# PrimeIntellect-ai/prime

Measured on AMD Instinct MI355X. Metric: tokens_per_sec, higher is better.
Workload: dtype bf16; 1 GPU; model=intellect_10b, global_batch=8, seq_len=2048, parallelism=diloco1_h100_int8ring

## Files before the change

### prime_amd/ops/csrc/attention.hip

```cpp
#include "common.h"
#include <stdlib.h>
#include <type_traits>

typedef __attribute__((ext_vector_type(8))) short short8;
typedef __attribute__((ext_vector_type(4))) float f32x4;
typedef __attribute__((address_space(3))) char lds_char;
typedef __attribute__((address_space(3))) void lds_void;
typedef __attribute__((address_space(1))) const void g_void;

__device__ __forceinline__ short8 ld8(const bf16* p) {
  return *reinterpret_cast<const short8*>(p);
}

__device__ __forceinline__ f32x4 mfma16(short8 a, short8 b, f32x4 c) {
  return __builtin_amdgcn_mfma_f32_16x16x32_bf16(a, b, c, 0, 0, 0);
}

__device__ __forceinline__ float grp16_max(float x) {
#pragma unroll
  for (int off = 1; off < 16; off <<= 1) x = fmaxf(x, __shfl_xor(x, off, 64));
  return x;
}
__device__ __forceinline__ float grp16_sum(float x) {
#pragma unroll
  for (int off = 1; off < 16; off <<= 1) x += __shfl_xor(x, off, 64);
  return x;
}

#define NEG_INF (-1e30f)


template <int ROWS, int COLS, int NT = 256>
__device__ __forceinline__ void stage_tile(const bf16* __restrict__ gbase,
                                           int64_t row_stride, bf16* lds_tile,
                                           int tid) {
  constexpr int UNITS = ROWS * COLS / 8;
  constexpr int UPR = COLS / 8;
  static_assert(UNITS % NT == 0, "tile not divisible by block lanes");
#pragma unroll
  for (int i = 0; i < UNITS / NT; ++i) {
    const int u = i * NT + tid;
    const int row = u / UPR;
    const int colb = ((u % UPR) * 16) ^ ((row & 7) << 4);
    const bf16* src = gbase + (int64_t)row * row_stride + colb / 2;
    const int wid = tid >> 6;
    lds_void* dst = (lds_void*)((lds_char*)lds_tile + i * (NT * 16) + wid * 1024);
    __builtin_amdgcn_global_load_lds((g_void*)src, dst, 16, 0, 0);
  }
}

template <int COLS>
__device__ __forceinline__ short8 ld8_swz(const bf16* lds_tile, int row,
                                          int colb) {
  return *reinterpret_cast<const short8*>(
      reinterpret_cast<const char*>(lds_tile) + row * (COLS * 2) +
      (colb ^ ((row & 7) << 4)));
}

template <int COLS>
__device__ __forceinline__ void st16_swz(bf16* lds_tile, int row, int col,
                                         bf16 v) {
  *reinterpret_cast<bf16*>(reinterpret_cast<char*>(lds_tile) + row * (COLS * 2) +
                           ((col * 2) ^ ((row & 7) << 4))) = v;
}

__device__ __forceinline__ void wave_lds_fence() {
  asm volatile("s_waitcnt lgkmcnt(0)" ::: "memory");
  __builtin_amdgcn_sched_barrier(0);
}

__device__ __forceinline__ int doc_clamp(int v, int hi) {
  return v < 0 ? 0 : (v > hi ? hi : v);
}

template <int D, int NW, bool DOC = false>
__global__ __launch_bounds__(512) void flash_fwd_kernel(
    const bf16* __restrict__ Q, const bf16* __restrict__ K,
    const bf16* __restrict__ Vt, bf16* __restrict__ O, float* __restrict__ lse,
    int B, int H, int Hkv, int S, float scale, int causal,
    int64_t sqb, int64_t sqs, int64_t sqh,
    int64_t skb, int64_t sks, int64_t skh,
    const int* __restrict__ doc) {
  constexpr int DS = D / 32;
  constexpr int DT = D / 16;
  constexpr int QT = NW * 16;
  const int n_qt = S / QT;
  const int bh = blockIdx.x / n_qt;
  const int qt = n_qt - 1 - (blockIdx.x - bh * n_qt);
  const int b = bh / H, h = bh - b * H;
  const int hkv = h / (H / Hkv);
  const int wid = threadIdx.x >> 6;
  const int lane = threadIdx.x & 63;
  const int lg = lane >> 4, li = lane & 15;
  const int q0 = qt * QT + wid * 16;

  const bf16* Qb = Q + b * sqb + h * sqh;
  const bf16* Kb = K + b * skb + hkv * skh;
  const bf16* Vtb = Vt + ((int64_t)(b * Hkv + hkv) * D) * S;

  __shared__ bf16 k_lds[64 * D];
  __shared__ bf16 vt_lds[D * 64];
  __shared__ bf16 p_lds_all[NW][16 * 64];
  bf16* p_lds = p_lds_all[wid];

  short8 qf[DS];
#pragma unroll
  for (int ds = 0; ds < DS; ++ds)
    qf[ds] = ld8(Qb + (int64_t)(q0 + li) * sqs + ds * 32 + lg * 8);

  float m[4], l[4];
  f32x4 o_acc[DT];
#pragma unroll
  for (int r = 0; r < 4; ++r) { m[r] = NEG_INF; l[r] = 0.f; }
#pragma unroll
  for (int dt = 0; dt < DT; ++dt) o_acc[dt] = f32x4{0.f, 0.f, 0.f, 0.f};

  const int kv_end = causal ? (qt * QT + QT) : S;
  int kv_begin = 0, my_kv_begin = 0, row_ds[4];
  if (DOC) {
    const int* doc_b = doc + (int64_t)b * S;
    kv_begin = doc_clamp(doc_b[qt * QT], qt * QT) & ~63;
    my_kv_begin = doc_clamp(doc_b[q0], q0) & ~63;
#pragma unroll
    for (int r = 0; r < 4; ++r) row_ds[r] = doc_b[q0 + lg * 4 + r];
  }
  for (int kv = kv_begin; kv < kv_end; kv += 64) {
    __syncthreads();
    stage_tile<64, D, NW * 64>(Kb + (int64_t)kv * sks, sks, k_lds, threadIdx.x);
    stage_tile<D, 64, NW * 64>(Vtb + kv, S, vt_lds, threadIdx.x);
    __syncthreads();
    if (DOC && kv < my_kv_begin) continue;

    f32x4 s[4];
#pragma unroll
    for (int sub = 0; sub < 4; ++sub) {
      f32x4 acc{0.f, 0.f, 0.f, 0.f};
#pragma unroll
      for (int ds = 0; ds < DS; ++ds)
        acc = mfma16(qf[ds], ld8_swz<D>(k_lds, sub * 16 + li, ds * 64 + lg * 16), acc);
      s[sub] = acc;
    }
    float alpha[4];
#pragma unroll
    for (int r = 0; r < 4; ++r) {
      const int qg = q0 + lg * 4 + r;
      float tmax = NEG_INF;
#pragma unroll
      for (int sub = 0; sub < 4; ++sub) {
        float v = s[sub][r] * scale;
        if (causal && (kv + sub * 16 + li) > qg) v = NEG_INF;
        if (DOC && (kv + sub * 16 + li) < row_ds[r]) v = NEG_INF;
        s[sub][r] = v;
        tmax = fmaxf(tmax, v);
      }
      tmax = grp16_max(tmax);
      const float mnew = fmaxf(m[r], tmax);
      alpha[r] = (mnew == m[r]) ? 1.f : __expf(m[r] - mnew);
      float psum = 0.f;
#pragma unroll
      for (int sub = 0; sub < 4; ++sub) {
        const float p = (DOC && s[sub][r] <= NEG_INF)
                            ? 0.f : __expf(s[sub][r] - mnew);
        s[sub][r] = p;
        psum += p;
      }
      l[r] = l[r] * alpha[r] + grp16_sum(psum);
      m[r] = mnew;
    }
    float amin = 1.f;
#pragma unroll
    for (int r = 0; r < 4; ++r) amin = fminf(amin, alpha[r]);
    if (__ballot(amin < 1.f)) {
#pragma unroll
      for (int dt = 0; dt < DT; ++dt)
#pragma unroll
        for (int r = 0; r < 4; ++r) o_acc[dt][r] *= alpha[r];
    }
#pragma unroll
    for (int sub = 0; sub < 4; ++sub)
#pragma unroll
      for (int r = 0; r < 4; ++r)
        st16_swz<64>(p_lds, lg * 4 + r, sub * 16 + li, f2bf(s[sub][r]));
    wave_lds_fence();
#pragma unroll
    for (int dt = 0; dt < DT; ++dt)
#pragma unroll
      for (int ks = 0; ks < 2; ++ks)
        o_acc[dt] = mfma16(ld8_swz<64>(p_lds, li, ks * 64 + lg * 16),
                           ld8_swz<64>(vt_lds, dt * 16 + li, ks * 64 + lg * 16),
                           o_acc[dt]);
  }
#pragma unroll
  for (int r = 0; r < 4; ++r) {
    const float inv = (l[r] > 0.f) ? 1.f / l[r] : 0.f;
    const int qg = q0 + lg * 4 + r;
    bf16* orow = O + (((int64_t)(b * S + qg)) * H + h) * D;
#pragma unroll
    for (int dt = 0; dt < DT; ++dt)
      orow[dt * 16 + li] = f2bf(o_acc[dt][r] * inv);
    if (li == 0)
      lse[((int64_t)(b * S + qg)) * H + h] = m[r] + __logf(fmaxf(l[r], 1e-30f));
  }
}


typedef __attribute__((ext_vector_type(16))) float f32x16;

__device__ __forceinline__ f32x16 mfma32(short8 a, short8 b, f32x16 c) {
  return __builtin_amdgcn_mfma_f32_32x32x16_bf16(a, b, c, 0, 0, 0);
}

__device__ __forceinline__ unsigned cvt_pk_bf16(float lo_, float hi_) {
  unsigned r;
  asm("v_cvt_pk_bf16_f32 %0, %1, %2" : "=v"(r) : "v"(lo_), "v"(hi_));
  return r;
}

__device__ __forceinline__ void permlane32_swap(unsigned& a, unsigned& b) {
  asm volatile("v_permlane32_swap_b32 %0, %1" : "+v"(a), "+v"(b));
}

template <int D, bool DOC = false>
__global__ __launch_bounds__(512, 2) void flash_fwd_v5_kernel(
    const bf16* __restrict__ Q, const bf16* __restrict__ K,
    const bf16* __restrict__ Vt, bf16* __restrict__ O, float* __restrict__ lse,
    int B, int H, int Hkv, int S, float scale, int causal,
    int64_t sqb, int64_t sqs, int64_t sqh,
    int64_t skb, int64_t sks, int64_t skh,
    const int* __restrict__ doc) {
  constexpr int DSL = D / 16;
  constexpr int DT32 = D / 32;
  const int n_qt = S / 256;
  const int nwg = gridDim.x;
  int vb = blockIdx.x;
  if ((nwg & 7) == 0) vb = (blockIdx.x & 7) * (nwg >> 3) + (blockIdx.x >> 3);
  const int bh = vb / n_qt;
  const int qt = n_qt - 1 - (vb - bh * n_qt);
  const int b = bh / H, h = bh - b * H;
  const int hkv = h / (H / Hkv);
  const int wid = threadIdx.x >> 6;
  const int lane = threadIdx.x & 63;
  const int lo = lane & 31, hi = lane >> 5;
  const int q0w = qt * 256 + wid * 32;

  const bf16* Qb = Q + b * sqb + h * sqh;
  const bf16* Kb = K + b * skb + hkv * skh;
  const bf16* Vtb = Vt + ((int64_t)(b * Hkv + hkv) * D) * S;

  __shared__ bf16 k_lds[2][64 * D];
  __shared__ bf16 vt_lds[2][D * 64];
  __shared__ float bcast_all[8][32];
  float* bcast = bcast_all[wid];

  short8 qf[DSL];
#pragma unroll
  for (int ds = 0; ds < DSL; ++ds) {
    const bf16* src = Qb + (int64_t)(q0w + lo) * sqs + ds * 16 + hi * 8;
    short8 raw = ld8(src);
    short8 sc;
#pragma unroll
    for (int j = 0; j < 8; ++j) {
      bf16 v = reinterpret_cast<const bf16*>(&raw)[j];
      reinterpret_cast<bf16*>(&sc)[j] = f2bf(bf2f(v) * scale);
    }
    qf[ds] = sc;
  }

  float m_run = NEG_INF, l_run = 0.f;
  f32x16 o_acc[DT32];
#pragma unroll
  for (int dt = 0; dt < DT32; ++dt)
#pragma unroll
    for (int r = 0; r < 16; ++r) o_acc[dt][r] = 0.f;

  const int kv_end = causal ? (qt * 256 + 256) : S;
  const int my_kv_end = causal ? (q0w + 32) : S;
  int kv_begin = 0, my_kv_begin = 0, my_ds = 0, my_ds_last = 0;
  if (DOC) {
    const int* doc_b = doc + (int64_t)b * S;
    kv_begin = doc_clamp(doc_b[qt * 256], qt * 256) & ~63;
    my_kv_begin = doc_clamp(doc_b[q0w], q0w) & ~63;
    my_ds = doc_b[q0w + lo];
    my_ds_last = doc_b[q0w + 31];
  }
  stage_tile<64, D, 512>(Kb + (int64_t)kv_begin * sks, sks, k_lds[0], threadIdx.x);
  stage_tile<D, 64, 512>(Vtb + kv_begin, S, vt_lds[0], threadIdx.x);
  int idx = 0;
  for (int kv = kv_begin, kt = 0; kv < kv_end; kv += 64, ++kt) {
    idx = kt % 2;
    __syncthreads();
    if (kv + 64 < kv_end) {
      stage_tile<64, D, 512>(Kb + (int64_t)(kv + 64) * sks, sks,
                             k_lds[(kt + 1) % 2], threadIdx.x);
      stage_tile<D, 64, 512>(Vtb + kv + 64, S, vt_lds[(kt + 1) % 2],
                             threadIdx.x);
    }
    if (kv >= my_kv_end) continue;
    if (DOC && kv < my_kv_begin) continue;

    f32x16 st[2];
#pragma unroll
    for (int t = 0; t < 2; ++t) {
#pragma unroll
      for (int r = 0; r < 16; ++r) st[t][r] = 0.f;
#pragma unroll
      for (int ds = 0; ds < DSL; ++ds) {
        const short8 kf = ld8_swz<D>(k_lds[idx], t * 32 + lo, ds * 32 + hi * 16);
        st[t] = mfma32(kf, qf[ds], st[t]);
      }
    }
    float tmax = NEG_INF;
    if (DOC && kv < my_ds_last) {
#pragma unroll
      for (int t = 0; t < 2; ++t)
#pragma unroll
        for (int r = 0; r < 16; ++r) {
          const int kg = kv + t * 32 + (r & 3) + 8 * (r >> 2) + 4 * hi;
          if (kg < my_ds) st[t][r] = NEG_INF;
        }
    }
#pragma unroll
    for (int t = 0; t < 2; ++t)
#pragma unroll
      for (int r = 0; r < 16; ++r) {
        const int kg = kv + t * 32 + (r & 3) + 8 * (r >> 2) + 4 * hi;
        if (causal && kg > q0w + lo) st[t][r] = NEG_INF;
        tmax = fmaxf(tmax, st[t][r]);
      }
    tmax = fmaxf(tmax, __shfl_xor(tmax, 32, 64));
    const float thr = 8.f;
    float alpha = 1.f;
    if (__ballot(tmax > m_run + thr)) {
      const float mnew = fmaxf(m_run, tmax);
      alpha = __expf(m_run - mnew);
      m_run = mnew;
      if (hi == 0) bcast[lo] = alpha;
      wave_lds_fence();
#pragma unroll
      for (int dt = 0; dt < DT32; ++dt)
#pragma unroll
        for (int r = 0; r < 16; ++r)
          o_acc[dt][r] *= bcast[(r & 3) + 8 * (r >> 2) + 4 * hi];
    }
    float psum = 0.f;
#pragma unroll
    for (int t = 0; t < 2; ++t)
#pragma unroll
      for (int r = 0; r < 16; ++r) {
        const float pv = (st[t][r] <= NEG_INF) ? 0.f : __expf(st[t][r] - m_run);
        st[t][r] = pv;
        psum += pv;
      }
    psum += __shfl_xor(psum, 32, 64);
    l_run = l_run * alpha + psum;

    short8 pa[2 * 2];
#pragma unroll
    for (int t = 0; t < 2; ++t) {
#pragma unroll
      for (int kst = 0; kst < 2; ++kst) {
        const int g0 = 4 * (2 * kst), g1 = 4 * (2 * kst + 1);
        unsigned x0 = cvt_pk_bf16(st[t][g0 + 0], st[t][g0 + 1]);
        unsigned x1 = cvt_pk_bf16(st[t][g0 + 2], st[t][g0 + 3]);
        unsigned y0 = cvt_pk_bf16(st[t][g1 + 0], st[t][g1 + 1]);
        unsigned y1 = cvt_pk_bf16(st[t][g1 + 2], st[t][g1 + 3]);
        permlane32_swap(x0, y0);
        permlane32_swap(x1, y1);
        short8 frag;
        reinterpret_cast<unsigned*>(&frag)[0] = x0;
        reinterpret_cast<unsigned*>(&frag)[1] = x1;
        reinterpret_cast<unsigned*>(&frag)[2] = y0;
        reinterpret_cast<unsigned*>(&frag)[3] = y1;
        pa[t * 2 + kst] = frag;
      }
    }
#pragma unroll
    for (int dt = 0; dt < DT32; ++dt)
#pragma unroll
      for (int ks = 0; ks < 4; ++ks)
        o_acc[dt] = mfma32(pa[ks],
                           ld8_swz<64>(vt_lds[idx], dt * 32 + lo, ks * 32 + hi * 16),
                           o_acc[dt]);
  }
  if (hi == 0) bcast[lo] = (l_run > 0.f) ? 1.f / l_run : 0.f;
  wave_lds_fence();
#pragma unroll
  for (int r = 0; r < 16; ++r) {
    const int qr = (r & 3) + 8 * (r >> 2) + 4 * hi;
    const float inv = bcast[qr];
    bf16* orow = O + (((int64_t)(b * S + q0w + qr)) * H + h) * D;
#pragma unroll
    for (int dt = 0; dt < DT32; ++dt)
      orow[dt * 32 + lo] = f2bf(o_acc[dt][r] * inv);
  }
  if (hi == 0)
    lse[((int64_t)(b * S + q0w + lo)) * H + h] = m_run + __logf(fmaxf(l_run, 1e-30f));
}

__global__ void attn_delta_kernel(const bf16* __restrict__ dO,
                                  const bf16* __restrict__ O,
                                  float* __restrict__ delta, int64_t rows,
                                  int D, const float* __restrict__ lse,
                                  float* __restrict__ rowc_t, int S, int H) {
  const int64_t row0 = (int64_t)blockIdx.x * (blockDim.x >> 6) + (threadIdx.x >> 6);
  const int lane = threadIdx.x & 63;
  for (int64_t r = row0; r < rows; r += (int64_t)gridDim.x * (blockDim.x >> 6)) {
    float acc = 0.f;
    for (int i = lane * 2; i < D; i += 128) {
      acc += bf2f(dO[r * D + i]) * bf2f(O[r * D + i]);
      acc += bf2f(dO[r * D + i + 1]) * bf2f(O[r * D + i + 1]);
    }
    acc = wave_reduce_sum(acc);
    if (lane == 0) {
      delta[r] = acc;
      if (rowc_t) {
        const int64_t bs = r / H;
        const int h = (int)(r - bs * H);
        const int64_t bb = bs / S;
        const int s = (int)(bs - bb * S);
        const int64_t t = (bb * H + h) * S + s;
        rowc_t[t] = lse[r];
        rowc_t[rows + t] = acc;
      }
    }
  }
}

template <int D>
__global__ __launch_bounds__(256) void attn_delta_dot_kernel(
    const bf16* __restrict__ dO, const bf16* __restrict__ O,
    const float* __restrict__ lse, float* __restrict__ delta,
    float* __restrict__ rowc_t, bf16* __restrict__ dOt, int S, int H,
    int64_t rows) {
  constexpr int LPR = D / 8;
  constexpr int RPP = 256 / LPR;
  constexpr int NP = 64 / RPP;
  constexpr int TPD = D + 8;
  __shared__ __attribute__((aligned(16))) bf16 tile[64][TPD];
  __shared__ float sdelta[64];
  int idx = blockIdx.x;
  const int h = idx % H; idx /= H;
  const int n_st = S / 64;
  const int st = idx % n_st;
  const int b = idx / n_st;
  const int t = threadIdx.x;
  const int m = t % LPR, rr = t / LPR;
  const int64_t tok0 = (int64_t)b * S + st * 64;
  const int64_t tcol = ((int64_t)b * H + h) * S + st * 64;

  short8 vdo[NP], vo[NP];
#pragma unroll
  for (int p = 0; p < NP; ++p) {
    const int64_t off = ((tok0 + p * RPP + rr) * H + h) * D + m * 8;
    vdo[p] = *reinterpret_cast<const short8*>(dO + off);
    vo[p] = *reinterpret_cast<const short8*>(O + off);
  }
  float lv = 0.f;
  if (t >= 64 && t < 128) lv = lse[(tok0 + (t - 64)) * H + h];

#pragma unroll
  for (int p = 0; p < NP; ++p) {
    const int row = p * RPP + rr;
    *reinterpret_cast<short8*>(&tile[row][m * 8]) = vdo[p];
    const bf16* a = reinterpret_cast<const bf16*>(&vdo[p]);
    const bf16* c = reinterpret_cast<const bf16*>(&vo[p]);
    float q[4];
#pragma unroll
    for (int i = 0; i < 4; ++i) {
      float acc = 0.f;
      acc += bf2f(a[2 * i]) * bf2f(c[2 * i]);
      acc += bf2f(a[2 * i + 1]) * bf2f(c[2 * i + 1]);
      q[i] = acc;
    }
#pragma unroll
    for (int i = 0; i < 4; ++i) {
      if (D == 64) q[i] = q[i] + 0.f;
      else q[i] += __shfl_down(q[i], 8, 64);
    }
#pragma unroll
    for (int off = 4; off > 0; off >>= 1)
#pragma unroll
      for (int i = 0; i < 4; ++i) q[i] += __shfl_down(q[i], off, 64);
    if (m == 0) sdelta[row] = (q[0] + q[2]) + (q[1] + q[3]);
  }
  __syncthreads();
  if (t < 64) {
    const float d = sdelta[t];
    delta[(tok0 + t) * H + h] = d;
    rowc_t[rows + tcol + t] = d;
  } else if (t < 128) {
    rowc_t[tcol + (t - 64)] = lv;
  }
  bf16* dbase = dOt + ((int64_t)b * H + h) * D * S + st * 64;
#pragma unroll
  for (int i = 0; i < D / 32; ++i) {
    const int u = i * 256 + t;
    const int d = u >> 3, s8 = (u & 7) * 8;
    short8 v;
#pragma unroll
    for (int j = 0; j < 8; ++j)
      reinterpret_cast<short*>(&v)[j] =
          reinterpret_cast<const short*>(&tile[s8 + j][d])[0];
    *reinterpret_cast<short8*>(dbase + (int64_t)d * S + s8) = v;
  }
}

template <int D, bool DOC = false>
__global__ __launch_bounds__(512, 2) void flash_bwd_dq_v5_kernel(
    const bf16* __restrict__ Q, const bf16* __restrict__ K,
    const bf16* __restrict__ V, const bf16* __restrict__ Kt,
    const bf16* __restrict__ dO, const float* __restrict__ lse,
    const float* __restrict__ delta, bf16* __restrict__ dQ, int B, int H,
    int Hkv, int S, float scale, int causal,
    int64_t sqb, int64_t sqs, int64_t sqh,
    int64_t skb, int64_t sks, int64_t skh,
    int64_t svb, int64_t svs, int64_t svh,
    const int* __restrict__ doc) {
  constexpr int DSL = D / 16;
  constexpr int DT32 = D / 32;
  const int n_qt = S / 256;
  const int nwg = gridDim.x;
  int vb = blockIdx.x;
  if ((nwg & 7) == 0) vb = (blockIdx.x & 7) * (nwg >> 3) + (blockIdx.x >> 3);
  const int bh = vb / n_qt;
  const int qt = n_qt - 1 - (vb - bh * n_qt);
  const int b = bh / H, h = bh - b * H;
  const int hkv = h / (H / Hkv);
  const int wid = threadIdx.x >> 6;
  const int lane = threadIdx.x & 63;
  const int lo = lane & 31, hi = lane >> 5;
  const int q0w = qt * 256 + wid * 32;

  const bf16* Qb = Q + b * sqb + h * sqh;
  const bf16* Kb = K + b * skb + hkv * skh;
  const bf16* Vb = V + b * svb + hkv * svh;
  const bf16* Ktb = Kt + ((int64_t)(b * Hkv + hkv) * D) * S;
  const bf16* dOb = dO + ((int64_t)b * S * H + h) * D;
  const float* lse_b = lse + (int64_t)b * S * H + h;
  const float* dl_b = delta + (int64_t)b * S * H + h;

  __shared__ bf16 k_lds[2][64 * D];
  __shared__ bf16 v_lds[2][64 * D];
  __shared__ bf16 kt_lds[2][D * 64];

  short8 qf[DSL], dof[DSL];
#pragma unroll
  for (int ds = 0; ds < DSL; ++ds) {
    const bf16* src = Qb + (int64_t)(q0w + lo) * sqs + ds * 16 + hi * 8;
    short8 raw = ld8(src);
    short8 sc;
#pragma unroll
    for (int j = 0; j < 8; ++j) {
      bf16 v = reinterpret_cast<const bf16*>(&raw)[j];
      reinterpret_cast<bf16*>(&sc)[j] = f2bf(bf2f(v) * scale);
    }
    qf[ds] = sc;
    dof[ds] = ld8(dOb + (int64_t)(q0w + lo) * H * D + ds * 16 + hi * 8);
  }
  const float lse_q = lse_b[(int64_t)(q0w + lo) * H];
  const float dl_q = dl_b[(int64_t)(q0w + lo) * H];

  f32x16 dq_acc[DT32];
#pragma unroll
  for (int dt = 0; dt < DT32; ++dt)
#pragma unroll
    for (int r = 0; r < 16; ++r) dq_acc[dt][r] = 0.f;

  const int kv_end = causal ? (qt * 256 + 256) : S;
  const int my_kv_end = causal ? (q0w + 32) : S;
  int kv_begin = 0, my_kv_begin = 0, my_ds = 0;
  if (DOC) {
    const int* doc_b = doc + (int64_t)b * S;
    kv_begin = doc_clamp(doc_b[qt * 256], qt * 256) & ~63;
    my_kv_begin = doc_clamp(doc_b[q0w], q0w) & ~63;
    my_ds = doc_b[q0w + lo];
  }
  stage_tile<64, D, 512>(Kb + (int64_t)kv_begin * sks, sks, k_lds[0], threadIdx.x);
  stage_tile<64, D, 512>(Vb + (int64_t)kv_begin * svs, svs, v_lds[0], threadIdx.x);
  stage_tile<D, 64, 512>(Ktb + kv_begin, S, kt_lds[0], threadIdx.x);
  int idx = 0;
  for (int kv = kv_begin; kv < kv_end; kv += 64, idx ^= 1) {
    __syncthreads();
    if (kv + 64 < kv_end) {
      stage_tile<64, D, 512>(Kb + (int64_t)(kv + 64) * sks, sks,
                             k_lds[idx ^ 1], threadIdx.x);
      stage_tile<64, D, 512>(Vb + (int64_t)(kv + 64) * svs, svs,
                             v_lds[idx ^ 1], threadIdx.x);
      stage_tile<D, 64, 512>(Ktb + kv + 64, S, kt_lds[idx ^ 1], threadIdx.x);
    }
    if (kv >= my_kv_end) continue;
    if (DOC && kv < my_kv_begin) continue;

    f32x16 st[2], dpt[2];
#pragma unroll
    for (int t = 0; t < 2; ++t) {
#pragma unroll
      for (int r = 0; r < 16; ++r) { st[t][r] = 0.f; dpt[t][r] = 0.f; }
#pragma unroll
      for (int ds = 0; ds < DSL; ++ds) {
        const short8 kf = ld8_swz<D>(k_lds[idx], t * 32 + lo, ds * 32 + hi * 16);
        const short8 vf = ld8_swz<D>(v_lds[idx], t * 32 + lo, ds * 32 + hi * 16);
        st[t] = mfma32(kf, qf[ds], st[t]);
        dpt[t] = mfma32(vf, dof[ds], dpt[t]);
      }
    }
#pragma unroll
    for (int t = 0; t < 2; ++t)
#pragma unroll
      for (int r = 0; r < 16; ++r) {
        const int kg = kv + t * 32 + (r & 3) + 8 * (r >> 2) + 4 * hi;
        float p = __expf(st[t][r] - lse_q);
        if (causal && kg > q0w + lo) p = 0.f;
        if (DOC && kg < my_ds) p = 0.f;
        st[t][r] = p * (dpt[t][r] - dl_q) * scale;
      }
    short8 da[2 * 2];
#pragma unroll
    for (int t = 0; t < 2; ++t) {
#pragma unroll
      for (int kst = 0; kst < 2; ++kst) {
        const int g0 = 4 * (2 * kst), g1 = 4 * (2 * kst + 1);
        unsigned x0 = cvt_pk_bf16(st[t][g0 + 0], st[t][g0 + 1]);
        unsigned x1 = cvt_pk_bf16(st[t][g0 + 2], st[t][g0 + 3]);
        unsigned y0 = cvt_pk_bf16(st[t][g1 + 0], st[t][g1 + 1]);
        unsigned y1 = cvt_pk_bf16(st[t][g1 + 2], st[t][g1 + 3]);
        permlane32_swap(x0, y0);
        permlane32_swap(x1, y1);
        short8 frag;
        reinterpret_cast<unsigned*>(&frag)[0] = x0;
        reinterpret_cast<unsigned*>(&frag)[1] = x1;
        reinterpret_cast<unsigned*>(&frag)[2] = y0;
        reinterpret_cast<unsigned*>(&frag)[3] = y1;
        da[t * 2 + kst] = frag;
      }
    }
#pragma unroll
    for (int dt = 0; dt < DT32; ++dt)
#pragma unroll
      for (int ks = 0; ks < 4; ++ks)
        dq_acc[dt] = mfma32(da[ks],
                            ld8_swz<64>(kt_lds[idx], dt * 32 + lo, ks * 32 + hi * 16),
                            dq_acc[dt]);
  }
#pragma unroll
  for (int r = 0; r < 16; ++r) {
    const int qr = (r & 3) + 8 * (r >> 2) + 4 * hi;
    bf16* row = dQ + (((int64_t)(b * S + q0w + qr)) * H + h) * D;
#pragma unroll
    for (int dt = 0; dt < DT32; ++dt)
      row[dt * 32 + lo] = f2bf(dq_acc[dt][r]);
  }
}

template <int D, bool DOC = false>
__global__ __launch_bounds__(256) void flash_bwd_dq_kernel(
    const bf16* __restrict__ Q, const bf16* __restrict__ K,
    const bf16* __restrict__ V, const bf16* __restrict__ Kt,
    const bf16* __restrict__ dO, const float* __restrict__ lse,
    const float* __restrict__ delta, bf16* __restrict__ dQ, int B, int H,
    int Hkv, int S, float scale, int causal,
    int64_t sqb, int64_t sqs, int64_t sqh,
    int64_t skb, int64_t sks, int64_t skh,
    int64_t svb, int64_t svs, int64_t svh,
    const int* __restrict__ doc) {
  constexpr int DS = D / 32;
  constexpr int DT = D / 16;
  const int n_qt = S / 64;
  const int bh = blockIdx.x / n_qt;
  const int qt = n_qt - 1 - (blockIdx.x - bh * n_qt);
  const int b = bh / H, h = bh - b * H;
  const int hkv = h / (H / Hkv);
  const int wid = threadIdx.x >> 6;
  const int lane = threadIdx.x & 63;
  const int lg = lane >> 4, li = lane & 15;
  const int q0 = qt * 64 + wid * 16;

  const bf16* Qb = Q + b * sqb + h * sqh;
  const bf16* Kb = K + b * skb + hkv * skh;
  const bf16* Vb = V + b * svb + hkv * svh;
  const bf16* Ktb = Kt + ((int64_t)(b * Hkv + hkv) * D) * S;
  const bf16* dOb = dO + ((int64_t)b * S * H + h) * D;
  const float* lse_b = lse + (int64_t)b * S * H + h;
  const float* dl_b = delta + (int64_t)b * S * H + h;

  __shared__ bf16 k_lds[64 * D];
  __shared__ bf16 v_lds[64 * D];
  __shared__ bf16 kt_lds[D * 64];
  __shared__ bf16 ds_lds_all[4][16 * 64];
  bf16* ds_lds = ds_lds_all[wid];

  short8 qf[DS], dof[DS];
#pragma unroll
  for (int ds = 0; ds < DS; ++ds) {
    qf[ds] = ld8(Qb + (int64_t)(q0 + li) * sqs + ds * 32 + lg * 8);
    dof[ds] = ld8(dOb + (int64_t)(q0 + li) * H * D + ds * 32 + lg * 8);
  }
  float lse_r[4], dl_r[4];
#pragma unroll
  for (int r = 0; r < 4; ++r) {
    lse_r[r] = lse_b[(int64_t)(q0 + lg * 4 + r) * H];
    dl_r[r] = dl_b[(int64_t)(q0 + lg * 4 + r) * H];
  }
  f32x4 dq_acc[DT];
#pragma unroll
  for (int dt = 0; dt < DT; ++dt) dq_acc[dt] = f32x4{0.f, 0.f, 0.f, 0.f};

  const int kv_end = causal ? (qt * 64 + 64) : S;
  int kv_begin = 0, my_kv_begin = 0, row_ds[4];
  if (DOC) {
    const int* doc_b = doc + (int64_t)b * S;
    kv_begin = doc_clamp(doc_b[qt * 64], qt * 64) & ~63;
    my_kv_begin = doc_clamp(doc_b[q0], q0) & ~63;
#pragma unroll
    for (int r = 0; r < 4; ++r) row_ds[r] = doc_b[q0 + lg * 4 + r];
  }
  for (int kv = kv_begin; kv < kv_end; kv += 64) {
    __syncthreads();
    stage_tile<64, D>(Kb + (int64_t)kv * sks, sks, k_lds, threadIdx.x);
    stage_tile<64, D>(Vb + (int64_t)kv * svs, svs, v_lds, threadIdx.x);
    stage_tile<D, 64>(Ktb + kv, S, kt_lds, threadIdx.x);
    __syncthreads();
    if (DOC && kv < my_kv_begin) continue;
#pragma unroll
    for (int sub = 0; sub < 4; ++sub) {
      f32x4 s_acc{0.f, 0.f, 0.f, 0.f}, dp_acc{0.f, 0.f, 0.f, 0.f};
#pragma unroll
      for (int ds = 0; ds < DS; ++ds) {
        s_acc = mfma16(qf[ds], ld8_swz<D>(k_lds, sub * 16 + li, ds * 64 + lg * 16), s_acc);
        dp_acc = mfma16(dof[ds], ld8_swz<D>(v_lds, sub * 16 + li, ds * 64 + lg * 16), dp_acc);
      }
#pragma unroll
      for (int r = 0; r < 4; ++r) {
        const int qg = q0 + lg * 4 + r;
        const int kg = kv + sub * 16 + li;
        float p = __expf(s_acc[r] * scale - lse_r[r]);
        if (causal && kg > qg) p = 0.f;
        if (DOC && kg < row_ds[r]) p = 0.f;
        st16_swz<64>(ds_lds, lg * 4 + r, sub * 16 + li,
                     f2bf(p * (dp_acc[r] - dl_r[r]) * scale));
      }
    }
    wave_lds_fence();
#pragma unroll
    for (int dt = 0; dt < DT; ++dt)
#pragma unroll
      for (int ks = 0; ks < 2; ++ks)
        dq_acc[dt] = mfma16(ld8_swz<64>(ds_lds, li, ks * 64 + lg * 16),
                            ld8_swz<64>(kt_lds, dt * 16 + li, ks * 64 + lg * 16),
                            dq_acc[dt]);
  }
#pragma unroll
  for (int r = 0; r < 4; ++r) {
    bf16* row = dQ + (((int64_t)(b * S + q0 + lg * 4 + r)) * H + h) * D;
#pragma unroll
    for (int dt = 0; dt < DT; ++dt) row[dt * 16 + li] = f2bf(dq_acc[dt][r]);
  }
}

template <int D, int NW, int DBUF, bool DOC>
__global__ __launch_bounds__(512) void flash_bwd_dkv_kernel(
    const bf16* __restrict__ Q, const bf16* __restrict__ Qt,
    const bf16* __restrict__ K, const bf16* __restrict__ V,
    const bf16* __restrict__ dO, const bf16* __restrict__ dOt,
    const float* __restrict__ rowc,
    float* __restrict__ wsK, float* __restrict__ wsV,
    bf16* __restrict__ dK, bf16* __restrict__ dV, int B, int H, int Hkv,
    int S, float scale, int causal, int splits, int direct,
    int64_t sqb, int64_t sqs, int64_t sqh,
    int64_t skb, int64_t sks, int64_t skh,
    int64_t svb, int64_t svs, int64_t svh,
    const int* __restrict__ doc_end) {
  static_assert((NW == 8 && DBUF == 2) || (NW == 4 && DBUF == 1),
                "only the two measured dK/dV shapes are built");
  constexpr int DS = D / 32;
  constexpr int DT = D / 16;
  const int n_kt = S / (NW * 16);
  const bool paired = direct && causal;
  const int per_bh = paired ? (n_kt + 1) / 2 : n_kt;
  const int per_split = (B * Hkv) * per_bh;
  const int blk_split = blockIdx.x / per_split;
  const int rem = blockIdx.x - blk_split * per_split;
  const int bh = rem / per_bh;
  const int kt0 = rem - bh * per_bh;
  const int n_pass = (paired && kt0 != n_kt - 1 - kt0) ? 2 : 1;
  const int b = bh / Hkv, hkv = bh - b * Hkv;
  const int group = H / Hkv;
  const int wid = threadIdx.x >> 6;
  const int lane = threadIdx.x & 63;
  const int lg = lane >> 4, li = lane & 15;

  const bf16* Kb = K + b * skb + hkv * skh;
  const bf16* Vb = V + b * svb + hkv * svh;
  const float* lse_t = rowc + (int64_t)b * H * S;
  const float* dl_t = lse_t + (int64_t)B * H * S;

  __shared__ bf16 q_lds[DBUF][64 * D];
  __shared__ bf16 do_lds[DBUF][64 * D];
  __shared__ bf16 qt_lds[DBUF][D * 64];
  __shared__ bf16 dot_lds[DBUF][D * 64];
  __shared__ bf16 pt_lds_all[NW][16 * 64];
  __shared__ bf16 dst_lds_all[NW][16 * 64];
  bf16* pt_lds = pt_lds_all[wid];
  bf16* dst_lds = dst_lds_all[wid];

  const int n_vs = direct ? splits : 1;
  for (int pv = 0; pv < n_pass * n_vs; ++pv) {
  const int pass = pv / n_vs;
  const int vs = pv - pass * n_vs;
  const int split = direct ? vs : blk_split;
  const int kt = pass ? n_kt - 1 - kt0 : kt0;
  const int k0 = kt * (NW * 16) + wid * 16;
  if (pv) __syncthreads();

  short8 kf[DS], vf[DS];
#pragma unroll
  for (int ds = 0; ds < DS; ++ds) {
    kf[ds] = ld8(Kb + (int64_t)(k0 + li) * sks + ds * 32 + lg * 8);
    vf[ds] = ld8(Vb + (int64_t)(k0 + li) * svs + ds * 32 + lg * 8);
  }
  f32x4 dk_acc[DT], dv_acc[DT];
#pragma unroll
  for (int dt = 0; dt < DT; ++dt) {
    dk_acc[dt] = f32x4{0.f, 0.f, 0.f, 0.f};
    dv_acc[dt] = f32x4{0.f, 0.f, 0.f, 0.f};
  }

  const int q_start = (causal ? (kt * (NW * 16)) / 64 * 64 : 0) + split * 64;
  int q_end = S, my_q_end = S, key_end4[4] = {S, S, S, S};
  if (DOC) {
    const int* de_b = doc_end + (int64_t)b * S;
    q_end = (doc_clamp(de_b[kt * (NW * 16) + NW * 16 - 1], S) + 63) & ~63;
    my_q_end = doc_clamp(de_b[k0 + 15], S);
#pragma unroll
    for (int r = 0; r < 4; ++r) key_end4[r] = doc_end[(int64_t)b * S + k0 + lg * 4 + r];
  }
  const int tiles_per_g =
      (q_end > q_start) ? (q_end - q_start + 64 * splits - 1) / (64 * splits) : 0;
  const int n_iter = group * tiles_per_g;
  const auto stage_it = [&](int it, int buf) {
    const int g_ = it / tiles_per_g;
    const int q0g_ = q_start + (it - g_ * tiles_per_g) * 64 * splits;
    const int h_ = hkv * group + g_;
    const bf16* Qb_ = Q + b * sqb + h_ * sqh;
    const bf16* dOb_ = dO + ((int64_t)b * S * H + h_) * D;
    const bf16* Qtb_ = Qt + ((int64_t)(b * H + h_) * D) * S;
    const bf16* dOtb_ = dOt + ((int64_t)(b * H + h_) * D) * S;
    stage_tile<64, D, NW * 64>(Qb_ + (int64_t)q0g_ * sqs, sqs, q_lds[buf], threadIdx.x);
    stage_tile<64, D, NW * 64>(dOb_ + (int64_t)q0g_ * H * D, (int64_t)H * D, do_lds[buf], threadIdx.x);
    stage_tile<D, 64, NW * 64>(Qtb_ + q0g_, S, qt_lds[buf], threadIdx.x);
    stage_tile<D, 64, NW * 64>(dOtb_ + q0g_, S, dot_lds[buf], threadIdx.x);
  };
  if (DBUF == 2 && n_iter > 0) stage_it(0, 0);
  for (int it = 0; it < n_iter; ++it) {
    const int g = it / tiles_per_g;
    const int q0g = q_start + (it - g * tiles_per_g) * 64 * splits;
    const int cur = (DBUF == 2) ? (it & 1) : 0;
    {
      __syncthreads();
      if (DBUF == 2) {
        if (it + 1 < n_iter) stage_it(it + 1, cur ^ 1);
      } else {
        stage_it(it, 0);
        __syncthreads();
      }
      const bool skip = (causal && q0g + 64 <= k0) || (DOC && q0g >= my_q_end);
      if (skip) continue;
#pragma unroll
      for (int sub = 0; sub < 4; ++sub) {
        f32x4 st_acc{0.f, 0.f, 0.f, 0.f}, dpt_acc{0.f, 0.f, 0.f, 0.f};
#pragma unroll
        for (int ds = 0; ds < DS; ++ds) {
          const short8 qb = ld8_swz<D>(q_lds[cur], sub * 16 + li, ds * 64 + lg * 16);
          const short8 dob = ld8_swz<D>(do_lds[cur], sub * 16 + li, ds * 64 + lg * 16);
          st_acc = mfma16(kf[ds], qb, st_acc);
          dpt_acc = mfma16(vf[ds], dob, dpt_acc);
        }
        const int qg = q0g + sub * 16 + li;
        const int64_t o = (int64_t)(hkv * group + g) * S + qg;
        const float lse_q = lse_t[o];
        const float dl_q = dl_t[o];
#pragma unroll
        for (int r = 0; r < 4; ++r) {
          float p = __expf(st_acc[r] * scale - lse_q);
          if (causal && k0 + lg * 4 + r > qg) p = 0.f;
          if (DOC && qg >= key_end4[r]) p = 0.f;
          st16_swz<64>(pt_lds, lg * 4 + r, sub * 16 + li, f2bf(p));
          st16_swz<64>(dst_lds, lg * 4 + r, sub * 16 + li,
                       f2bf(p * (dpt_acc[r] - dl_q) * scale));
        }
      }
      wave_lds_fence();
#pragma unroll
      for (int dt = 0; dt < DT; ++dt)
#pragma unroll
        for (int ks = 0; ks < 2; ++ks) {
          const short8 pa = ld8_swz<64>(pt_lds, li, ks * 64 + lg * 16);
          const short8 da = ld8_swz<64>(dst_lds, li, ks * 64 + lg * 16);
          dv_acc[dt] = mfma16(pa, ld8_swz<64>(dot_lds[cur], dt * 16 + li, ks * 64 + lg * 16), dv_acc[dt]);
          dk_acc[dt] = mfma16(da, ld8_swz<64>(qt_lds[cur], dt * 16 + li, ks * 64 + lg * 16), dk_acc[dt]);
        }
    }
  }
#pragma unroll
  for (int r = 0; r < 4; ++r) {
    const int kr = k0 + lg * 4 + r;
    const int64_t ob = (((int64_t)b * S + kr) * Hkv + hkv) * D + li;
    const int64_t wb = ((((int64_t)blk_split * B + b) * Hkv + hkv) * S + kr) * D + li;
#pragma unroll
    for (int dt = 0; dt < DT; ++dt) {
      if (direct) {
        float sk = 0.f + dk_acc[dt][r], sv = 0.f + dv_acc[dt][r];
        if (vs > 0) {
          sk = wsK[wb + dt * 16] + dk_acc[dt][r];
          sv = wsV[wb + dt * 16] + dv_acc[dt][r];
        }
        if (vs + 1 < n_vs) {
          wsK[wb + dt * 16] = sk;
          wsV[wb + dt * 16] = sv;
        } else {
          dK[ob + dt * 16] = f2bf(sk);
          dV[ob + dt * 16] = f2bf(sv);
        }
      } else {
        wsK[wb + dt * 16] = dk_acc[dt][r];
        wsV[wb + dt * 16] = dv_acc[dt][r];
      }
    }
  }
  }
}

__global__ void dkv_reduce_kernel(const float* __restrict__ wsK,
                                  const float* __restrict__ wsV,
                                  bf16* __restrict__ dK, bf16* __restrict__ dV,
                                  int B, int Hkv, int S, int D, int splits) {
  const int64_t n = (int64_t)B * Hkv * S * D;
  for (int64_t i = (int64_t)blockIdx.x * blockDim.x + threadIdx.x; i < n;
       i += (int64_t)gridDim.x * blockDim.x) {
    float k = 0.f, v = 0.f;
    for (int sp = 0; sp < splits; ++sp) {
      k += wsK[(int64_t)sp * n + i];
      v += wsV[(int64_t)sp * n + i];
    }
    const int d = (int)(i % D);
    int64_t r = i / D;
    const int sq = (int)(r % S);
    r /= S;
    const int hk = (int)(r % Hkv);
    const int bb = (int)(r / Hkv);
    const int64_t o = (((int64_t)(bb * S + sq)) * Hkv + hk) * D + d;
    dK[o] = f2bf(k);
    dV[o] = f2bf(v);
  }
}

template <typename To, typename From>
static To kernel_arg(From v) {
  static_assert(std::is_pointer<To>::value == std::is_pointer<From>::value,
                "pointer / scalar mismatch in a kernel argument list");
  return (To)v;
}

template <typename... P, typename... A>
static int attn_launch(void (*kernel)(P...), int64_t grid, int block,
                       hipStream_t stream, A... args) {
  hipLaunchKernelGGL(kernel, dim3((int)grid), dim3(block), 0, stream,
                     kernel_arg<P>(args)...);
  return (int)hipGetLastError();
}

#define BY_D_DOC(LAUNCH)                                          \
  (D == 128 ? (doc ? LAUNCH(128, true) : LAUNCH(128, false))      \
            : (doc ? LAUNCH(64, true) : LAUNCH(64, false)))

static bool attn_use_v5(int64_t S) {
  static const char* v5env = getenv("PRIME_ATTN_V5");
  return (S % 256 == 0) && !(v5env && v5env[0] == '0');
}

PRIME_API int prime_flash_fwd(hipStream_t stream, const void* Q, const void* K,
                              const void* Vt, void* O, void* lse, int64_t B,
                              int64_t H, int64_t Hkv, int64_t S, int64_t D,
                              double scale, int64_t causal,
                              int64_t sqb, int64_t sqs, int64_t sqh,
                              int64_t skb, int64_t sks, int64_t skh,
                              const void* doc_start) {
  if (S % 64 != 0 || (D != 64 && D != 128)) return hipErrorInvalidValue;
  const bool doc = doc_start != nullptr;
  if (doc && !causal) return hipErrorInvalidValue;
  const bool v5 = attn_use_v5(S);
#define FWD(DD, DOCV)                                                        \
  attn_launch(v5 ? flash_fwd_v5_kernel<DD, DOCV>                             \
                 : flash_fwd_kernel<DD, 4, DOCV>,                            \
              B * H * (S / (v5 ? 256 : 64)), v5 ? 512 : 256, stream, Q, K,   \
              Vt, O, lse, B, H, Hkv, S, scale, causal, sqb, sqs, sqh, skb,   \
              sks, skh, doc_start)
  return BY_D_DOC(FWD);
#undef FWD
}

PRIME_API int prime_attn_delta_t(hipStream_t stream, const void* dO,
                                 const void* O, const void* lse, void* delta,
                                 void* rowc_t, int64_t B, int64_t S, int64_t H,
                                 int64_t D) {
  if (!lse || !rowc_t) return hipErrorInvalidValue;
  const int64_t rows = B * S * H;
  int grid = prime_grid(rows * 64, 256);
  hipLaunchKernelGGL(attn_delta_kernel, dim3(grid), dim3(256), 0, stream,
                     (const bf16*)dO, (const bf16*)O, (float*)delta, rows,
                     (int)D, (const float*)lse, (float*)rowc_t, (int)S, (int)H);
  return (int)hipGetLastError();
}

PRIME_API int prime_attn_delta_dot(hipStream_t stream, const void* dO,
                                   const void* O, const void* lse, void* delta,
                                   void* rowc_t, void* dOt, int64_t B,
                                   int64_t S, int64_t H, int64_t D) {
  if (!dO || !O || !lse || !delta || !rowc_t || !dOt) return hipErrorInvalidValue;
  if (S % 64 != 0 || (D != 64 && D != 128)) return hipErrorInvalidValue;
  const int64_t rows = B * S * H;
  const int64_t grid = B * H * (S / 64);
  if (grid > 0x7fffffff) return hipErrorInvalidValue;
  if (grid == 0) return (int)hipSuccess;
  if (D == 64)
    hipLaunchKernelGGL(attn_delta_dot_kernel<64>, dim3((int)grid), dim3(256), 0,
                       stream, (const bf16*)dO, (const bf16*)O,
                       (const float*)lse, (float*)delta, (float*)rowc_t,
                       (bf16*)dOt, (int)S, (int)H, rows);
  else
    hipLaunchKernelGGL(attn_delta_dot_kernel<128>, dim3((int)grid), dim3(256),
                       0, stream, (const bf16*)dO, (const bf16*)O,
                       (const float*)lse, (float*)delta, (float*)rowc_t,
                       (bf16*)dOt, (int)S, (int)H, rows);
  return (int)hipGetLastError();
}

PRIME_API int prime_flash_bwd_dq(hipStream_t stream, const void* Q,
                                 const void* K, const void* V, const void* Kt,
                                 const void* dO, const void* lse,
                                 const void* delta, void* dQ, int64_t B,
                                 int64_t H, int64_t Hkv, int64_t S, int64_t D,
                                 double scale, int64_t causal,
                                 int64_t sqb, int64_t sqs, int64_t sqh,
                                 int64_t skb, int64_t sks, int64_t skh,
                                 int64_t svb, int64_t svs, int64_t svh,
                                 const void* doc_start) {
  if (S % 64 != 0 || (D != 64 && D != 128)) return hipErrorInvalidValue;
  const bool doc = doc_start != nullptr;
  if (doc && !causal) return hipErrorInvalidValue;
  const bool v5 = attn_use_v5(S);
#define DQ(DD, DOCV)                                                         \
  attn_launch(v5 ? flash_bwd_dq_v5_kernel<DD, DOCV>                          \
                 : flash_bwd_dq_kernel<DD, DOCV>,                            \
              B * H * (S / (v5 ? 256 : 64)), v5 ? 512 : 256, stream, Q, K,   \
              V, Kt, dO, lse, delta, dQ, B, H, Hkv, S, scale, causal, sqb,   \
              sqs, sqh, skb, sks, skh, svb, svs, svh, doc_start)
  return BY_D_DOC(DQ);
#undef DQ
}

static int64_t dkv_tile_rows(int64_t S) { return (S % 128 == 0) ? 128 : 64; }

PRIME_API int prime_flash_bwd_dkv_direct(int64_t B, int64_t Hkv, int64_t S,
                                         int64_t D, int64_t causal,
                                         int64_t has_doc) {
  const char* env = getenv("PRIME_ATTN_DKV_DIRECT");
  if (env && env[0] == '1') return 1;
  if (env && env[0] == '0') return 0;
  static int n_cu = 0;
  if (n_cu == 0) {
    int dev = 0, n = 0;
    if (hipGetDevice(&dev) != hipSuccess ||
        hipDeviceGetAttribute(&n, hipDeviceAttributeMultiprocessorCount, dev) != hipSuccess ||
        n <= 0)
      n = 256;
    n_cu = n;
  }
  const int64_t n_kt = S / dkv_tile_rows(S);
  const int64_t blocks = B * Hkv * (causal ? (n_kt + 1) / 2 : n_kt);
  return blocks >= n_cu ? 1 : 0;
}

PRIME_API int prime_flash_bwd_dkv(hipStream_t stream, const void* Q,
                                  const void* Qt, const void* K, const void* V,
                                  const void* dO, const void* dOt,
                                  const void* rowc, void* dK,
                                  void* dV, void* wsK, void* wsV,
                                  int64_t splits, int64_t B, int64_t H,
                                  int64_t Hkv, int64_t S, int64_t D,
                                  double scale, int64_t causal,
                                  int64_t sqb, int64_t sqs, int64_t sqh,
                                  int64_t skb, int64_t sks, int64_t skh,
                                  int64_t svb, int64_t svs, int64_t svh,
                                  const void* doc_end) {
  if (S % 64 != 0 || (D != 64 && D != 128)) return hipErrorInvalidValue;
  const bool doc = doc_end != nullptr;
  if (doc && !causal) return hipErrorInvalidValue;
  const bool direct =
      prime_flash_bwd_dkv_direct(B, Hkv, S, D, causal, doc) != 0;
  if (splits < 1) return hipErrorInvalidValue;
  if ((!direct || splits > 1) && (!wsK || !wsV)) return hipErrorInvalidValue;
  if (!rowc) return hipErrorInvalidValue;
  const bool nw8 = dkv_tile_rows(S) == 128;
  const int64_t n_kt = S / dkv_tile_rows(S);
  const int64_t per_bh = (direct && causal) ? (n_kt + 1) / 2 : n_kt;
#define DKV(DD, DOCV)                                                        \
  attn_launch(nw8 ? flash_bwd_dkv_kernel<DD, 8, 2, DOCV>                     \
                  : flash_bwd_dkv_kernel<DD, 4, 1, DOCV>,                    \
              B * Hkv * per_bh * (direct ? 1 : splits), nw8 ? 512 : 256,     \
              stream, Q, Qt, K, V, dO, dOt, rowc, wsK, wsV, dK, dV, B, H,    \
              Hkv, S, scale, causal, splits, direct, sqb, sqs, sqh, skb,     \
              sks, skh, svb, svs, svh, doc_end)
  int err = BY_D_DOC(DKV);
#undef DKV
  if (err || direct) return err;
  int rgrid = prime_grid(B * Hkv * S * D, 256);
  hipLaunchKernelGGL(dkv_reduce_kernel, dim3(rgrid), dim3(256), 0, stream,
                     (const float*)wsK, (const float*)wsV, (bf16*)dK,
                     (bf16*)dV, (int)B, (int)Hkv, (int)S, (int)D, (int)splits);
  return (int)hipGetLastError();
}
```

Measured before the change: 17420 tokens/s.

## Skip causal masking on interior tiles and pack bf16 LDS stores via DPP

Forward and backward attention kernels now apply the causal mask only on KV tiles that cross the diagonal, so interior tiles skip per-element index compares. The forward softmax drops the per-element -inf select and instead substitutes a zero max when the running max is still -inf in the document-masked case. The dK/dV kernel packs P and dS into bf16 pairs, exchanges them between neighbouring lanes with a DPP swap, and writes 32-bit LDS stores in place of 16-bit scalar stores. The aim is fewer VALU and LDS instructions, at the cost of more intricate lane shuffling that must match the swizzled layout exactly.

Measured after the change: 17640 tokens/s (median of 6 runs). 1.01x the previous value.

```diff
diff --git a/prime_amd/ops/csrc/attention.hip b/prime_amd/ops/csrc/attention.hip
--- a/prime_amd/ops/csrc/attention.hip
+++ b/prime_amd/ops/csrc/attention.hip
@@ -62,6 +62,13 @@
                                          bf16 v) {
   *reinterpret_cast<bf16*>(reinterpret_cast<char*>(lds_tile) + row * (COLS * 2) +
                            ((col * 2) ^ ((row & 7) << 4))) = v;
+}
+
+template <int COLS>
+__device__ __forceinline__ void st32_swz(bf16* lds_tile, int row, int col,
+                                         unsigned v) {
+  *reinterpret_cast<unsigned*>(reinterpret_cast<char*>(lds_tile) + row * (COLS * 2) +
+                               ((col * 2) ^ ((row & 7) << 4))) = v;
 }
 
 __device__ __forceinline__ void wave_lds_fence() {
@@ -218,6 +225,10 @@
 
 __device__ __forceinline__ void permlane32_swap(unsigned& a, unsigned& b) {
   asm volatile("v_permlane32_swap_b32 %0, %1" : "+v"(a), "+v"(b));
+}
+
+__device__ __forceinline__ unsigned lane_xor1(unsigned x) {
+  return (unsigned)__builtin_amdgcn_update_dpp((int)x, (int)x, 0xB1, 0xF, 0xF, false);
 }
 
 template <int D, bool DOC = false>
@@ -319,14 +330,19 @@
           if (kg < my_ds) st[t][r] = NEG_INF;
         }
     }
+    if (causal && kv + 63 > q0w) {
+#pragma unroll
+      for (int t = 0; t < 2; ++t)
+#pragma unroll
+        for (int r = 0; r < 16; ++r) {
+          const int kg = kv + t * 32 + (r & 3) + 8 * (r >> 2) + 4 * hi;
+          if (kg > q0w + lo) st[t][r] = NEG_INF;
+        }
+    }
 #pragma unroll
     for (int t = 0; t < 2; ++t)
 #pragma unroll
-      for (int r = 0; r < 16; ++r) {
-        const int kg = kv + t * 32 + (r & 3) + 8 * (r >> 2) + 4 * hi;
-        if (causal && kg > q0w + lo) st[t][r] = NEG_INF;
-        tmax = fmaxf(tmax, st[t][r]);
-      }
+      for (int r = 0; r < 16; ++r) tmax = fmaxf(tmax, st[t][r]);
     tmax = fmaxf(tmax, __shfl_xor(tmax, 32, 64));
     const float thr = 8.f;
     float alpha = 1.f;
@@ -342,12 +358,14 @@
         for (int r = 0; r < 16; ++r)
           o_acc[dt][r] *= bcast[(r & 3) + 8 * (r >> 2) + 4 * hi];
     }
+    float m_sub = m_run;
+    if (DOC && m_run <= NEG_INF) m_sub = 0.f;
     float psum = 0.f;
 #pragma unroll
     for (int t = 0; t < 2; ++t)
 #pragma unroll
       for (int r = 0; r < 16; ++r) {
-        const float pv = (st[t][r] <= NEG_INF) ? 0.f : __expf(st[t][r] - m_run);
+        const float pv = __expf(st[t][r] - m_sub);
         st[t][r] = pv;
         psum += pv;
       }
@@ -604,13 +622,22 @@
         dpt[t] = mfma32(vf, dof[ds], dpt[t]);
       }
     }
+    if (!DOC && causal && kv + 63 > q0w) {
+#pragma unroll
+      for (int t = 0; t < 2; ++t)
+#pragma unroll
+        for (int r = 0; r < 16; ++r) {
+          const int kg = kv + t * 32 + (r & 3) + 8 * (r >> 2) + 4 * hi;
+          if (kg > q0w + lo) st[t][r] = NEG_INF;
+        }
+    }
 #pragma unroll
     for (int t = 0; t < 2; ++t)
 #pragma unroll
       for (int r = 0; r < 16; ++r) {
         const int kg = kv + t * 32 + (r & 3) + 8 * (r >> 2) + 4 * hi;
         float p = __expf(st[t][r] - lse_q);
-        if (causal && kg > q0w + lo) p = 0.f;
+        if (DOC && causal && kg > q0w + lo) p = 0.f;
         if (DOC && kg < my_ds) p = 0.f;
         st[t][r] = p * (dpt[t][r] - dl_q) * scale;
       }
@@ -879,15 +906,28 @@
         const int64_t o = (int64_t)(hkv * group + g) * S + qg;
         const float lse_q = lse_t[o];
         const float dl_q = dl_t[o];
+        float pv[4], dsv[4];
 #pragma unroll
         for (int r = 0; r < 4; ++r) {
           float p = __expf(st_acc[r] * scale - lse_q);
           if (causal && k0 + lg * 4 + r > qg) p = 0.f;
           if (DOC && qg >= key_end4[r]) p = 0.f;
-          st16_swz<64>(pt_lds, lg * 4 + r, sub * 16 + li, f2bf(p));
-          st16_swz<64>(dst_lds, lg * 4 + r, sub * 16 + li,
-                       f2bf(p * (dpt_acc[r] - dl_q) * scale));
+          pv[r] = p;
+          dsv[r] = p * (dpt_acc[r] - dl_q) * scale;
         }
+        const unsigned p01 = cvt_pk_bf16(pv[0], pv[1]), p23 = cvt_pk_bf16(pv[2], pv[3]);
+        const unsigned d01 = cvt_pk_bf16(dsv[0], dsv[1]), d23 = cvt_pk_bf16(dsv[2], dsv[3]);
+        const int odd = li & 1;
+        const unsigned pgot = lane_xor1(odd ? p01 : p23);
+        const unsigned dgot = lane_xor1(odd ? d01 : d23);
+        const unsigned pown = odd ? p23 : p01, down = odd ? d23 : d01;
+        const unsigned sel0 = odd ? 0x01000504u : 0x05040100u;
+        const unsigned sel1 = odd ? 0x03020706u : 0x07060302u;
+        const int prow = lg * 4 + 2 * odd, pcol = sub * 16 + (li & ~1);
+        st32_swz<64>(pt_lds, prow, pcol, __builtin_amdgcn_perm(pgot, pown, sel0));
+        st32_swz<64>(pt_lds, prow + 1, pcol, __builtin_amdgcn_perm(pgot, pown, sel1));
+        st32_swz<64>(dst_lds, prow, pcol, __builtin_amdgcn_perm(dgot, down, sel0));
+        st32_swz<64>(dst_lds, prow + 1, pcol, __builtin_amdgcn_perm(dgot, down, sel1));
       }
       wave_lds_fence();
 #pragma unroll
```
